# NoSuchThingAsRandom/EpidemicSimulator

Hardware: AMD Instinct MI355X
Metric: citizen-timesteps/sec (higher is better)
Workload: dtype u32 citizen word; u32 uniform vs ceil(q*2^32) (reference: f64 uniform; tolerance 2^-32 per draw); 1 GPU; uk64m: 64000000 citizens, 290000 Output Areas, 10 seeds, steps 1..667 of 5000, interventions on; seed=1592598545

## Files before the change

epidemicsimulator_amd/_lib.py:

```python
import ctypes as C
import os

_HERE = os.path.dirname(os.path.abspath(__file__))
LIB_PATH = os.environ.get("ESIM_LIB") or os.path.join(_HERE, "libesim.so")

OK = 0
ERRORS = {-1: "EINVAL", -2: "ENODEVICE", -3: "ENOMEM", -4: "ESTATE", -5: "ERANGE", -6: "ESIM", -7: "ETIMEDOUT"}

SUSCEPTIBLE, EXPOSED, INFECTED, RECOVERED, VACCINATED = range(5)
HOUSEHOLD, WORKPLACE, SCHOOL = range(3)
MASK_NONE, MASK_PUBLIC_TRANSPORT, MASK_EVERYWHERE = range(3)
NO_ROOM = 0xFFFFFFFF
FLAG_USES_PUBLIC_TRANSPORT = 1
FLAG_MASK_COMPLIANT = 2


class EsimError(RuntimeError):
    def __init__(self, code, text):
        super().__init__("libesim %s (%d): %s" % (ERRORS.get(code, "?"), code, text))
        self.code = code


class Params(C.Structure):
    _fields_ = [
# ... 8 lines not shown


_u32p, _u16p, _u8p, _i32p = (C.POINTER(C.c_uint32), C.POINTER(C.c_uint16),
                             C.POINTER(C.c_uint8), C.POINTER(C.c_int32))


class PopulationStruct(C.Structure):
    _fields_ = [
        ("n_citizens", C.c_uint32), ("n_buildings", C.c_uint32), ("n_areas", C.c_uint32),
        ("n_rooms", C.c_uint32), ("n_seeds", C.c_uint32),
        ("citizen_id_base", C.c_uint32), ("n_citizens_global", C.c_uint32),
        ("n_shared_buildings", C.c_uint32), ("n_shared_rooms", C.c_uint32),
        ("home_building", _u32p), ("work_building", _u32p), ("room", _u32p),
        ("flags", _u8p), ("age", _u16p), ("occupation", _u8p),
        ("building_area", _u32p), ("building_type", _u8p), ("room_building", _u32p),
        ("seeds", _u32p), ("shared_building_local", _i32p), ("shared_room_local", _i32p),
    ]


class StepResult(C.Structure):
    _fields_ = [(n, C.c_uint32) for n in (
        "time_step", "susceptible", "exposed", "infected", "recovered", "vaccinated",
        "exposures_building", "exposures_bus", "lockdown", "vaccination_active", "mask_status",
        "n_riders", "vaccinated_now", "eligible_count", "disease_exists", "reserved")]

    def as_dict(self):
        return {n: int(getattr(self, n)) for n, _ in self._fields_ if n != "reserved"}


RECORD_FIELDS = [n for n, _ in StepResult._fields_]


class SynthSpec(C.Structure):
    _fields_ = [
        ("n_citizens", C.c_uint32), ("n_areas", C.c_uint32), ("citizens_per_school", C.c_uint32),
        ("n_seeds", C.c_uint32), ("seed", C.c_uint64), ("area_jitter", C.c_double),
        ("p_public_transport", C.c_double), ("p_mask_compliant", C.c_double),
        ("p_work_from_home", C.c_double), ("p_teaching", C.c_double),
        ("household_buildings_median", C.c_double), ("household_buildings_sigma", C.c_double),
        ("p_area_without_households", C.c_double),
        ("workplace_buildings_median", C.c_double), ("workplace_buildings_sigma", C.c_double),
        ("p_area_without_workplaces", C.c_double),
        ("workplace_floor_median", C.c_double), ("workplace_floor_sigma", C.c_double),
        ("teacher_candidate_schools", C.c_uint32), ("reserved", C.c_uint32),
    ]


SYMBOLS = [
    "esim_default_params", "esim_create", "esim_upload_population", "esim_reset", "esim_restart", "esim_restart_seeded", "esim_get_seeds", "esim_step",
    "esim_run", "esim_set_pipeline", "esim_chunk_timing", "esim_enable_chunk_kernel_timing", "esim_chunk_kernel_timings", "esim_vax_chunk_stats", "esim_vax_repair_stats", "esim_pipeline_timing",
    "esim_comm_unique_id", "esim_comm_init_rccl", "esim_comm_init_callback", "esim_comm_set_timeout", "esim_debug_inject_error", "esim_comm_stats", "esim_run_sharded", "esim_shard_stats",
    "esim_read_records", "esim_synchronize",
    "esim_download_state", "esim_download_exposure_log", "esim_area_census", "esim_area_arrival", "esim_area_series", "esim_area_status_series", "esim_set_groups", "esim_group_census", "esim_group_series", "esim_ensemble_begin", "esim_ensemble_begin_arrival", "esim_ensemble_fold", "esim_ensemble_read", "esim_checkpoint_size", "esim_checkpoint_save", "esim_checkpoint_restore", "esim_enable_phase_timing", "esim_phase_timings",
    "esim_enable_kernel_timing", "esim_kernel_timings", "esim_set_small_step_limit", "esim_set_tiny_chunk_limit", "esim_small_kernel_timing", "esim_debug_counters",
    "esim_last_error", "esim_destroy",
    "esim_threshold_lut", "esim_synth_preset", "esim_synth_create", "esim_synth_create_shard", "esim_synth_free",
    "esim_shard_population", "esim_shard_cuts",
]

ALLREDUCE_FN = C.CFUNCTYPE(C.c_int, C.c_void_p, C.c_int, C.c_void_p, C.c_size_t)

_lib = None


def load():
    global _lib
    if _lib is not None:
        return _lib
    if not os.path.exists(LIB_PATH):
        raise ImportError(
            "libesim.so is not built (%s). Run `python -c 'import __graft_entry__ as g; g.build()'` "
            "or `make -C epidemicsimulator_amd/csrc`. There is no CPU fallback." % LIB_PATH)
    lib = C.CDLL(LIB_PATH)
    vp, pvp = C.c_void_p, C.POINTER(C.c_void_p)
    sig = {
        "esim_default_params": (None, [C.POINTER(Params)]),
        "esim_create": (C.c_int, [C.POINTER(Params), pvp]),
        "esim_upload_population": (C.c_int, [vp, C.POINTER(PopulationStruct)]),
        "esim_reset": (C.c_int, [vp]),
        "esim_restart": (C.c_int, [vp, C.POINTER(Params)]),
        "esim_restart_seeded": (C.c_int, [vp, C.POINTER(Params), _u32p, C.c_uint32]),
        "esim_get_seeds": (C.c_int, [vp, _u32p, C.c_uint32, _u32p]),
        "esim_step": (C.c_int, [vp, C.POINTER(StepResult)]),
        "esim_run": (C.c_int, [vp, C.c_uint32, C.c_int, C.POINTER(StepResult), C.POINTER(C.c_uint32)]),
        "esim_comm_unique_id": (C.c_int, [vp, C.c_size_t]),
        "esim_comm_init_rccl": (C.c_int, [vp, vp, C.c_size_t, C.c_int, C.c_int]),
        "esim_comm_init_callback": (C.c_int, [vp, ALLREDUCE_FN, vp, C.c_int, C.c_int]),
        "esim_comm_set_timeout": (C.c_int, [vp, C.c_double]),
        "esim_debug_inject_error": (C.c_int, [vp, C.c_int]),
        "esim_comm_stats": (C.c_int, [vp, C.POINTER(C.c_uint64)]),
        "esim_run_sharded": (C.c_int, [vp, C.c_uint32, C.POINTER(C.c_uint32)]),
        "esim_shard_stats": (C.c_int, [vp, C.POINTER(C.c_uint64), C.POINTER(C.c_uint64)]),
        "esim_set_pipeline": (C.c_int, [vp, C.c_int]),
        "esim_chunk_timing": (C.c_int, [vp, C.POINTER(C.c_double), C.POINTER(C.c_uint64), C.POINTER(C.c_uint64)]),
        "esim_enable_chunk_kernel_timing": (C.c_int, [vp, C.c_int]),
        "esim_chunk_kernel_timings": (C.c_int, [vp, C.POINTER(C.c_double), C.POINTER(C.c_uint64)]),
        "esim_vax_chunk_stats": (C.c_int, [vp, C.POINTER(C.c_uint64), C.POINTER(C.c_uint64)]),
        "esim_vax_repair_stats": (C.c_int, [vp, C.POINTER(C.c_uint64)]),
        "esim_pipeline_timing": (C.c_int, [vp, C.POINTER(C.c_double), C.POINTER(C.c_uint64), C.POINTER(C.c_uint64)]),
        "esim_read_records": (C.c_int, [vp, C.c_uint32, C.c_uint32, C.POINTER(StepResult)]),
        "esim_synchronize": (C.c_int, [vp]),
        "esim_download_state": (C.c_int, [vp, _u8p, _u16p, _u32p, _u8p, _u8p]),
        "esim_download_exposure_log": (C.c_int, [vp, _u32p, _u32p, _u8p, C.c_uint32, _u32p]),
        "esim_area_census": (C.c_int, [vp, C.c_int, _u32p]),
        "esim_area_arrival": (C.c_int, [vp, C.c_int, _u32p]),
        "esim_area_series": (C.c_int, [vp, C.c_int, C.c_uint32, C.c_uint32, C.c_uint32, _u32p]),
        "esim_area_status_series": (C.c_int, [vp, C.c_int, C.c_int, C.c_uint32, C.c_uint32, C.c_uint32, _u32p]),
        "esim_set_groups": (C.c_int, [vp, _u16p, C.c_uint32]),
        "esim_group_census": (C.c_int, [vp, _u32p]),
        "esim_group_series": (C.c_int, [vp, C.c_int, C.c_uint32, C.c_uint32, C.c_uint32, _u32p]),
        "esim_ensemble_begin": (C.c_int, [vp, C.c_int, C.c_uint32, C.c_uint32]),
        "esim_ensemble_begin_arrival": (C.c_int, [vp, C.c_int, C.c_uint32]),
        "esim_ensemble_fold": (C.c_int, [vp]),
        "esim_ensemble_read": (C.c_int, [vp, _u32p, _u32p, C.POINTER(C.c_uint64), C.POINTER(C.c_uint64)]),
        "esim_checkpoint_size": (C.c_int, [vp, C.POINTER(C.c_size_t)]),
        "esim_checkpoint_save": (C.c_int, [vp, vp, C.c_size_t]),
        "esim_checkpoint_restore": (C.c_int, [vp, vp, C.c_size_t]),
        "esim_enable_phase_timing": (C.c_int, [vp, C.c_int]),
        "esim_phase_timings": (C.c_int, [vp, C.POINTER(C.c_double)]),
        "esim_enable_kernel_timing": (C.c_int, [vp, C.c_int]),
        "esim_kernel_timings": (C.c_int, [vp, C.POINTER(C.c_double), C.POINTER(C.c_uint32)]),
        "esim_debug_counters": (C.c_int, [vp, C.POINTER(C.c_uint32)]),
        "esim_set_small_step_limit": (C.c_int, [vp, C.c_uint32]),
        "esim_set_tiny_chunk_limit": (C.c_int, [vp, C.c_uint32]),
        "esim_small_kernel_timing": (C.c_int, [vp, C.POINTER(C.c_double), C.POINTER(C.c_uint64)]),
        "esim_last_error": (C.c_char_p, [vp]),
        "esim_destroy": (None, [vp]),
        "esim_threshold_lut": (C.c_int, [C.POINTER(Params), C.POINTER(C.c_uint64)]),
        "esim_synth_preset": (C.c_int, [C.c_char_p, C.POINTER(SynthSpec)]),
        "esim_synth_create": (C.c_int, [C.POINTER(SynthSpec), C.POINTER(PopulationStruct)]),
        "esim_synth_create_shard": (C.c_int, [C.POINTER(SynthSpec), C.c_uint32, C.c_uint32, C.POINTER(PopulationStruct)]),
        "esim_shard_cuts": (C.c_int, [C.POINTER(PopulationStruct), C.c_uint32, C.c_int, C.POINTER(C.c_uint32)]),
        "esim_synth_free": (None, [C.POINTER(PopulationStruct)]),
        "esim_shard_population": (C.c_int, [C.POINTER(PopulationStruct), _u32p, C.c_uint32, C.c_uint32,
                                            C.POINTER(PopulationStruct)]),
    }
    for name, (res, args) in sig.items():
        fn = getattr(lib, name)
        fn.restype, fn.argtypes = res, args
    _lib = lib
    return lib


ESIM_OK, ESIM_ERANGE = 0, -5
AREA_CURRENT, AREA_HOME = 0, 1
SERIES_INFECTED, SERIES_EXPOSURES = 0, 1
BY_GROUP = 2
MAX_GROUPS = 1024
NEVER = 0xFFFFFFFF
GROUP_SERIES_EXPOSURES = 5
AREA_SERIES_INCIDENCE = 5
DEBUG_COUNTERS = ("t", "chunk_ok", "chunk_parallel", "chunk_pairs", "n_items", "items_per_wave", "n_units", "chunk_bus",
                  "n_route_pairs_big", "n_newexp", "log_len", "n_susceptible", "lockdown", "mask", "at_work", "bus_dir")
CHUNK_KERNELS = ("marks", "fold", "draw", "units", "count", "books", "scatter", "vax", "vax_adj", "vax_final", "decide", "future", "map_clear", "tiny", "vax_repair")
PHASE_OF_KERNEL = {"marks": "Generate Exposures", "fold": "Generate Exposures", "draw": "Apply Exposures", "units": "Apply Exposures"}
TINY_PHASE_SHARES = {"Generate Exposures": 0.10, "Apply Exposures": 0.40, "Apply Interventions": 0.50}


def check(code, ctx=None):
    if code != OK:
        text = load().esim_last_error(ctx)
        raise EsimError(code, text.decode() if text else "")


def default_params(**overrides):
    p = Params()
    load().esim_default_params(C.byref(p))
    for k, v in overrides.items():
        if not hasattr(p, k):
            raise AttributeError("esim_params has no field %r" % k)
        setattr(p, k, v)
    return p
```

epidemicsimulator_amd/csrc/esim_host_timing.h:

```cpp
extern "C" int esim_vax_chunk_stats(esim_ctx *ctx, uint64_t *steps, uint64_t *cuts)
{
    esim_ctx_impl *c = CTX(ctx); if (!c) return ESIM_EINVAL;
    if (steps) *steps = c->vax_chunk_steps;
    if (cuts) *cuts = c->vax_chunk_cuts;
    return ESIM_OK;
}

extern "C" int esim_vax_repair_stats(esim_ctx *ctx, uint64_t *repairs)
{
    esim_ctx_impl *c = CTX(ctx); if (!c) return ESIM_EINVAL;
    if (repairs) *repairs = c->vax_chunk_repairs;
    return ESIM_OK;
}

extern "C" int esim_chunk_timing(esim_ctx *ctx, double *total_ms, uint64_t *steps, uint64_t *chunks)
{
    esim_ctx_impl *c = CTX(ctx); if (!c) return ESIM_EINVAL;
    if (total_ms) *total_ms = c->tm.chunk_ms;
    if (steps) *steps = c->tm.chunk_steps;
    if (chunks) *chunks = c->tm.chunk_count;
    c->tm.chunk_ms = 0; c->tm.chunk_steps = 0; c->tm.chunk_count = 0;
    return ESIM_OK;
}

extern "C" int esim_enable_chunk_kernel_timing(esim_ctx *ctx, int enable)
{
    esim_ctx_impl *c = CTX(ctx); if (!c) return ESIM_EINVAL;
    if (int rc = drain(c)) return rc;
    c->tm.kdetail = enable != 0;
    c->tm.kd_used = 0;
    for (int i = 0; i < ESIM_CK_N; ++i) { c->tm.kd_ms[i] = 0; c->tm.kd_calls[i] = 0; }
    return ESIM_OK;
}

extern "C" int esim_chunk_kernel_timings(esim_ctx *ctx, double ms[ESIM_CK_N], uint64_t calls[ESIM_CK_N])
{
    esim_ctx_impl *c = CTX(ctx);
    if (!c || !ms || !calls) return ESIM_EINVAL;
    if (int rc = drain(c)) return rc;
    kd_resolve(c);
    for (int i = 0; i < ESIM_CK_N; ++i) { ms[i] = c->tm.kd_ms[i]; calls[i] = c->tm.kd_calls[i]; c->tm.kd_ms[i] = 0; c->tm.kd_calls[i] = 0; }
    return ESIM_OK;
}

extern "C" int esim_pipeline_timing(esim_ctx *ctx, double *mean_step_ms, uint64_t *steps_timed, uint64_t *steps_run)
{
    esim_ctx_impl *c = CTX(ctx); if (!c) return ESIM_EINVAL;
    if (int rc = drain(c)) return rc;
    double acc = 0;
    const size_t n = c->tm.pkev_used / 2;
    for (size_t i = 0; i < n; ++i) { float ms; HIP_TRY(c, hipEventElapsedTime(&ms, c->tm.pkev[2 * i], c->tm.pkev[2 * i + 1])); acc += ms; }
    if (mean_step_ms) *mean_step_ms = n ? acc / (double)n : 0.0;
    if (steps_timed) *steps_timed = n;
    if (steps_run) *steps_run = c->tm.pipe_steps;
    c->tm.pkev_used = 0; c->tm.pipe_steps = 0;
    return ESIM_OK;
}

extern "C" int esim_debug_counters(esim_ctx *ctx, uint32_t out[16])
{
    esim_ctx_impl *c = CTX(ctx);
    if (!c || !c->uploaded || !out) return ESIM_EINVAL;
    HIP_TRY(c, hipSetDevice(c->P.device));
    Ctrl h;
    const int rc = read_ctrl(c, &h);
    if (rc) return rc;
    const uint32_t v[16] = { h.t, h.chunk_ok, h.chunk_parallel, h.chunk_pairs, h.n_items, h.items_per_wave, h.n_units, h.chunk_bus,
                             h.n_route_pairs_big, h.n_newexp, h.log_len, h.n_susceptible, h.lockdown, h.mask, h.at_work, h.bus_dir };
    std::memcpy(out, v, sizeof v);
    return ESIM_OK;
}

#ifdef ESIM_COUNT_WORK
extern "C" int esim_work_counters(esim_ctx *ctx, unsigned long long *out, uint32_t n)
{
    esim_ctx_impl *c = CTX(ctx);
    if (!c || !c->uploaded || !out) return ESIM_EINVAL;
    if (int rc = drain(c)) return rc;
    unsigned long long h[WK_N];
    HIP_TRY(c, hipMemcpy(h, c->d.work_cnt, sizeof h, hipMemcpyDeviceToHost));
    HIP_TRY(c, hipMemset(c->d.work_cnt, 0, sizeof h));
    for (uint32_t i = 0; i < n; ++i) out[i] = i < WK_N ? h[i] : 0ull;
    return ESIM_OK;
}
#endif

#ifdef ESIM_WAVE_PROFILE
extern "C" int esim_prof_read(esim_ctx *ctx, uint32_t *out, uint32_t n_words, int *clock_khz)
{
    esim_ctx_impl *c = CTX(ctx);
    if (!c || !c->uploaded || !out) return ESIM_EINVAL;
    if (int rc = drain(c)) return rc;
    HIP_TRY(c, hipMemcpy(out, c->d.prof_buf, sizeof(uint32_t) * std::min<uint32_t>(n_words, 16384u * 16u), hipMemcpyDeviceToHost));
    if (clock_khz) HIP_TRY(c, hipDeviceGetAttribute(clock_khz, hipDeviceAttributeWallClockRate, c->P.device));
    return ESIM_OK;
}
#endif

extern "C" int esim_enable_phase_timing(esim_ctx *ctx, int enable)
{
    esim_ctx_impl *c = CTX(ctx); if (!c) return ESIM_EINVAL;
    c->tm.phase = enable != 0;
    return ESIM_OK;
}

extern "C" int esim_phase_timings(esim_ctx *ctx, double out[4])
{
    esim_ctx_impl *c = CTX(ctx);
    if (!c || !out) return ESIM_EINVAL;
    out[0] = c->tm.phase_s[0]; out[1] = c->tm.phase_s[1]; out[2] = c->tm.phase_s[2];
    out[3] = out[0] + out[1] + out[2];
    return ESIM_OK;
}

extern "C" int esim_enable_kernel_timing(esim_ctx *ctx, int enable)
{
    esim_ctx_impl *c = CTX(ctx); if (!c) return ESIM_EINVAL;
    c->tm.kernel = enable > 0;
    if (enable > 0) c->tm.stride = (uint32_t)enable;
    c->tm.kev_used = 0;
    if (enable > 0) {
        HIP_TRY(c, hipSetDevice(c->P.device));
// ... 28 lines not shown
```

epidemicsimulator_amd/csrc/esim_kernels_chunk.h:

```cpp
#pragma once
#define BF_WIN 1024
__device__ __forceinline__ void block_scan_1024(uint32_t *v, uint32_t *wtmp)
{
    const uint32_t tid = threadIdx.x, lane = tid & 63u, wv = tid >> 6;
    uint32_t x = v[tid];
#pragma unroll
    for (int o = 1; o < 64; o <<= 1) { const uint32_t y = __shfl_up(x, o, 64); if (lane >= (uint32_t)o) x += y; }
    if (lane == 63u) wtmp[wv] = x;
    __syncthreads();
    if (tid == 0) { uint32_t a = 0; for (uint32_t w = 0; w < FIN_TPB / 64; ++w) { const uint32_t y = wtmp[w]; wtmp[w] = a; a += y; } }
    __syncthreads();
    v[tid] = x + wtmp[wv];
    __syncthreads();
}

__device__ __forceinline__ void future_body(const Dev &d, uint32_t max_ahead, uint32_t limit_t, uint32_t *win, uint32_t *wtmp)
{
    Ctrl *ctrl = d.ctrl;
    const uint32_t t0 = ld(&ctrl->t), tid = threadIdx.x;
    const uint32_t n_ahead = t0 > limit_t ? 0u : (limit_t - t0 + 1u < max_ahead ? limit_t - t0 + 1u : max_ahead);
    const int et = (int)d.exposed_time, it = (int)d.infected_time;
    const int base_idx = (int)(t0 + TE_BIAS) - et - 1 - it;
    { const int k = base_idx + (int)tid; win[tid] = (k >= 0 && k < (int)TE_SLOTS) ? ld(&d.hist[k]) : 0u; }
    __syncthreads();
// ... 1136 lines not shown
{
    ItemFetch f;
    f.slot = FX(x, LANE_HSLOT); f.id = FX(x, 0); f.a_lo = FX(x, 1); f.a_hi = FX(x, 2); f.b_lo = FX(x, 3); f.b_hi = FX(x, 4); f.aux = FX(x, 5); f.link = FX(x, 6);
    f.c0 = 0u; f.c1 = 0u;
    if (f.slot < d.hcap) {
        item_counts(d, x, f.slot, lane, n, AW, BUS, f.c0, f.c1);
        iv_count(FX(x, 7), lane, AW, BUS, f.c0, f.c1);
    }
    return f;
}

__device__ __forceinline__ bool item_ok(const Dev &d, const ItemFetch &it)
{
    if (it.slot >= d.hcap) return false;
    if (it.id < d.n_bld) return it.a_lo <= it.a_hi && it.a_hi <= d.n && it.b_lo <= it.b_hi && it.b_hi <= d.n_wrk_idx;
    if (it.id < d.n_bld + d.n_room) return it.a_lo <= it.a_hi && it.a_hi <= d.n_room_idx && (it.link == 0xFFFFFFFFu || it.link < d.hcap);
    return true;
}
#define PAIR_SPREAD 1237u
__device__ __forceinline__ void route_pair_small(const Dev &d, Ctrl *ctrl, const ChunkShared &sm, uint32_t off, uint32_t sz, uint32_t j, uint32_t t0, uint32_t lane WORK_ARG)
{
    const uint64_t seed = ((uint64_t)d.seed_hi << 32) | d.seed_lo;
    const uint32_t s = t0 + j, mask = sm.dec[j].mask;
    uint32_t c = 0, w = 0, key = 0;
    bool inf = false;
    WORK_ADD(WK_ROUTE_PAIRS, lane == 0 ? 1 : 0); WORK_ADD(WK_RIDERS, lane < sz ? 1 : 0);
    bool can = false;
    if (lane < sz) {
        c = d.route_riders[off + lane];
        w = d.cit[c];
        inf = status_in_chunk(d, w, t0, j) == ESIM_INFECTED;
        const uint32_t te = CW_TE(w);
        can = !(w <= CW_MAKE(s + TE_BIAS, CW_BUS_EXPOSED | (w & CW_KEEP)) || (te >= TE_RECOVERED && te != TE_SUSCEPTIBLE) || j > CW_VAX_REL(w));
    }
    if (!__any(inf) || !__any(can)) return;
    uint32_t rank = 0;
    if (sz > d.bus_capacity) {
        if (lane < sz) key = philox4x32_10(d.id_base + c, s, ESIM_SLOT_BUS_ORDER, 0u, d.seed_lo, d.seed_hi).w0;
        for (uint32_t i = 0; i < sz; ++i) {
            const uint32_t ki = (uint32_t)__builtin_amdgcn_readlane((int)key, (int)i);
            rank += ki < key || (ki == key && i < lane);
        }
    }
    const uint32_t bus = rank / d.bus_capacity;
    const unsigned long long inf_m = __ballot(inf);
    uint32_t k = 0;
    const uint32_t n_bus = (sz + d.bus_capacity - 1u) / d.bus_capacity;
    for (uint32_t b = 0; b < n_bus; ++b) {
        const unsigned long long on_b = __ballot(lane < sz && bus == b);
        if (bus == b) k = (uint32_t)__popcll(on_b & inf_m);
    }
    if (lane < sz && k && can) {
        const uint32_t row = (!(w & FL_MASK_COMPLIANT) && mask == ESIM_MASK_EVERYWHERE) ? 1u : 0u;
        WORK_ADD(WK_BUS_DRAWS, 1);
        if (esim_u32(seed, d.id_base + c, s, ESIM_SLOT_BUS) < sm.thr[row * 256u + (k & 255u)]) { WORK_ADD(WK_HITS, 1); expose_min(d, ctrl, c, w, s, CW_BUS_EXPOSED); }
    }
}

template <uint32_t NT>
__device__ __forceinline__ void route_pair_big(const Dev &d, Ctrl *ctrl, const ChunkShared &sm, RouteShared &rs, uint32_t code, uint32_t t0, uint32_t n WORK_ARG)
{
    const uint64_t seed = ((uint64_t)d.seed_hi << 32) | d.seed_lo;
    const uint32_t r = code >> 7, j = code & 127u;
    if (r >= d.n_routes || j >= n) { if (threadIdx.x == 0) ctrl->error = (uint32_t)(-ESIM_ERANGE); return; }
    const uint32_t off = d.route_off[r], sz = d.route_off[r + 1] - off;
    if (sz > CHUNK_ROUTE_MAX) { if (threadIdx.x == 0) ctrl->error = (uint32_t)(-ESIM_ERANGE); return; }
    const uint32_t s = t0 + j, mask = sm.dec[j].mask;
    WORK_ADD(WK_ROUTE_PAIRS, threadIdx.x == 0 ? 1 : 0);
    int loc_inf = 0, loc_can = 0;
    for (uint32_t i = threadIdx.x; i < sz; i += NT) {
        const uint32_t c = d.route_riders[off + i];
        WORK_ADD(WK_RIDERS, 1);
        const uint32_t w = d.cit[c], te = CW_TE(w);
        rs.s_inf[i] = status_in_chunk(d, w, t0, j) == ESIM_INFECTED ? 1 : 0;
        loc_inf |= rs.s_inf[i];
        loc_can |= !(w <= CW_MAKE(s + TE_BIAS, CW_BUS_EXPOSED | (w & CW_KEEP)) || (te >= TE_RECOVERED && te != TE_SUSCEPTIBLE) || j > CW_VAX_REL(w)) ? 1 : 0;
    }
    const int any_inf = __syncthreads_or(loc_inf), any_can = __syncthreads_or(loc_can);
    if (!any_inf || !any_can) return;
    for (uint32_t i = threadIdx.x; i < sz; i += NT)
        rs.s_key[i] = philox4x32_10(d.id_base + d.route_riders[off + i], s, ESIM_SLOT_BUS_ORDER, 0u, d.seed_lo, d.seed_hi).w0;
    for (uint32_t i = threadIdx.x; i < sz / d.bus_capacity + 1u; i += NT) rs.s_cnt[i] = 0u;
    __syncthreads();
    for (uint32_t i = threadIdx.x; i < sz; i += NT) {
        const uint32_t ki = rs.s_key[i];
        uint32_t rank = 0;
        for (uint32_t qq = 0; qq < sz; ++qq) { const uint32_t kq = rs.s_key[qq]; rank += kq < ki || (kq == ki && qq < i); }
        const uint32_t bus = rank / d.bus_capacity;
        rs.s_bus[i] = (uint16_t)bus;
        if (rs.s_inf[i]) atomicAdd(&rs.s_cnt[bus], 1u);
    }
    __syncthreads();
    for (uint32_t i = threadIdx.x; i < sz; i += NT) {
        const uint32_t k = rs.s_cnt[rs.s_bus[i]];
        if (!k) continue;
        const uint32_t c = d.route_riders[off + i];
        const uint32_t w = d.cit[c], te = CW_TE(w);
        if (w <= CW_MAKE(s + TE_BIAS, CW_BUS_EXPOSED | (w & CW_KEEP)) || (te >= TE_RECOVERED && te != TE_SUSCEPTIBLE) || j > CW_VAX_REL(w)) continue;
        const uint32_t row = (!(w & FL_MASK_COMPLIANT) && mask == ESIM_MASK_EVERYWHERE) ? 1u : 0u;
        WORK_ADD(WK_BUS_DRAWS, 1);
        if (esim_u32(seed, d.id_base + c, s, ESIM_SLOT_BUS) < sm.thr[row * 256u + (k & 255u)]) { WORK_ADD(WK_HITS, 1); expose_min(d, ctrl, c, w, s, CW_BUS_EXPOSED); }
    }
    __syncthreads();
}

__global__ __launch_bounds__(TPB) void k_chunk_draw(Dev d, uint32_t n_mw)
// ... 69 lines not shown
        if (v + 1u < d_hi) sl_cur = fetch_slot(d, FX(id_cur, LANE_HSLOT), lane);
        const uint32_t pq0 = PROF_NOW();
        const ItemFetch it = decode_item(d, x, lane, n, AW, BUS);
        if (it.slot == ITEM_UNUSED) continue;
        if (!item_ok(d, it)) { if (lane == 0) RAISE(ctrl, ESIM_ERANGE, ERR_AT_ITEM_CHECK); continue; }
        if (it.id >= route_base) continue;
        const uint32_t pi0 = PROF_NOW();
        pst[0] += pi0 - pq0;
        (void)pi0; ++p_items; WORK_ADD(WK_ITEMS, lane == 0 ? 1 : 0);
        if (it.id < d.n_bld) {
            if (it.aux == ESIM_SCHOOL) continue;
            const uint32_t n_res = it.a_hi - it.a_lo, n_wrk = it.b_hi - it.b_lo;
            uint32_t rm = 0u, wm = 0u, rw = 0u, ww = 0u;
            if (lane < n_res) rm = d.res_idx ? d.res_idx[it.a_lo + lane] : it.a_lo + lane;
            if (lane < n_wrk) wm = d.wrk_idx[it.b_lo + lane];
            if (lane < n_res) rw = d.cit[rm];
            if (lane < n_wrk) ww = d.cit[wm];
            const uint32_t pq1 = PROF_NOW();
            const uint32_t S = item_steps_regs(it.c0, it.c1, lane, ws, t0, AW, EV);
            __builtin_amdgcn_wave_barrier();
            const uint32_t pq2 = PROF_NOW();
            const UnitSrc src = { it.slot, it.link, FX(x, 7) };
            list_or_units(d, ctrl, sm, ws, d.res_idx, it.a_lo, it.a_hi, src, lane, 0u, S, t0 WORK_PASS, true, rm, rw);
            const uint32_t pq3 = PROF_NOW();
            list_or_units(d, ctrl, sm, ws, d.wrk_idx, it.b_lo, it.b_hi, src, lane, 1u, S, t0 WORK_PASS, true, wm, ww);
            const uint32_t pq4 = PROF_NOW();
            pst[1] += pq1 - pi0; pst[2] += pq2 - pq1; pst[3] += pq3 - pq2; pst[4] += pq4 - pq3;
        } else {
            const uint32_t n_mem = it.a_hi - it.a_lo;
            uint32_t mm = 0u, mw = 0u;
            if (lane < n_mem) mm = d.room_idx[it.a_lo + lane];
            school_counts(d, it.link, lane, n, q0, q1, ws);
            if (lane < n_mem) mw = d.cit[mm];
            const uint32_t S = item_steps_regs(it.c0, it.c1, lane, ws, t0, AW, EV);
            __builtin_amdgcn_wave_barrier();
            const UnitSrc src = { it.slot, it.link, FX(x, 7) };
            list_or_units(d, ctrl, sm, ws, d.room_idx, it.a_lo, it.a_hi, src, lane, 2u, S, t0 WORK_PASS, true, mm, mw);
        }
        __builtin_amdgcn_wave_barrier();
        { const uint32_t dt = PROF_NOW() - pi0; p_item_max = dt > p_item_max ? dt : p_item_max; }
    }
    const uint32_t pt2 = PROF_NOW();
    for (uint32_t k0 = 0; k0 * G < K; k0 += 64u) {
        if (k0) {
            const uint32_t kk = (k0 + lane) * G + w_rep;
            have = false;
            if (kk < K) {
                const uint32_t src = (w_base + n_mw - (uint32_t)(((unsigned long long)kk * PAIR_SPREAD) % n_mw)) % n_mw;
                code_l = d.route_pairs[(size_t)src * K + kk];
                have = kk < d.pair_cnt[src] && (code_l >> 7) < d.n_routes && (code_l & 127u) < n;
            }
            if (have) { const uint32_t r = code_l >> 7; off_l = d.route_off[r]; sz_l = d.route_off[r + 1] - off_l; }
        }
        unsigned long long todo = __ballot(have);
        while (todo) {
            const int src_lane = __ffsll((long long)todo) - 1;
            todo &= todo - 1ull;
            const uint32_t code = __shfl(code_l, src_lane, 64), off = __shfl(off_l, src_lane, 64), sz = __shfl(sz_l, src_lane, 64);
            route_pair_small(d, ctrl, sm, off, sz, code & 127u, t0, lane WORK_PASS);
        }
    }
    WORK_FLUSH(d);
    const uint32_t pt3 = PROF_NOW();
#ifndef ESIM_PROFILE_UNITS
    PROF_PUT(d, 0, pt0); PROF_PUT(d, 1, pt1); PROF_PUT(d, 2, pt2); PROF_PUT(d, 3, pt3);
    PROF_PUT(d, 4, p_items); PROF_PUT(d, 5, p_item_max); PROF_PUT(d, 6, wsc[threadIdx.x >> 6].rounds);
    PROF_PUT(d, 11, pst[0]); PROF_PUT(d, 12, pst[1]); PROF_PUT(d, 13, pst[2]); PROF_PUT(d, 14, pst[3]); PROF_PUT(d, 15, pst[4]);
#endif
    (void)pst;
    (void)pt0; (void)pt1; (void)pt2; (void)pt3; (void)p_items; (void)p_item_max;
}

__global__ __launch_bounds__(TPB) void k_chunk_units(Dev d)
{
    __shared__ ChunkShared sm;
    __shared__ WaveScratch wsc[TPB / 64];
    __shared__ RouteShared rs;
    Ctrl *ctrl = d.ctrl;
    const uint32_t t0 = ctrl->chunk_t0, n = ctrl->chunk_ok;
    if (!ctrl->chunk_parallel || n == 0u) return;
    const uint32_t lane = threadIdx.x & 63u;
    const uint32_t wave = (blockIdx.x * TPB + threadIdx.x) >> 6, n_waves = (gridDim.x * TPB) >> 6;
    const uint32_t pu0 = PROF_NOW();
    WORK_TALLY;
    uint32_t pu_n = 0u, pu_max = 0u, pu_it = 0u;
    const uint32_t qr = wave & (SUBQ - 1u), first = wave / SUBQ, step = n_waves / SUBQ;
    const uint32_t n_units = step ? min(ld(&d.hot[(HOT_UNITS + qr) * HOT_STRIDE]), d.unit_qcap) : 0u;
    const uint32_t n_pairs = min(ld(&d.hot[HOT_BIGPAIRS * HOT_STRIDE]), d.big_pairs_cap);
    if (__syncthreads_or(first < n_units) == 0 && n_pairs == 0u) return;
    for (uint32_t i = threadIdx.x; i < n; i += TPB) sm.dec[i] = d.dec[i];
    for (uint32_t i = threadIdx.x; i < 512u; i += TPB) sm.thr[i] = d.thr[i];
    __syncthreads();
    WaveScratch &ws = wsc[threadIdx.x >> 6];
    const uint32_t *q_words = reinterpret_cast<const uint32_t *>(d.units + (size_t)qr * d.unit_qcap);
    const Decision q0 = lane < n ? sm.dec[lane] : Decision{ 0u, 0u, 0u, 0u };
    const Decision q1 = 64u + lane < n ? sm.dec[64u + lane] : Decision{ 0u, 0u, 0u, 0u };
    M96 AW, BUS;
    schedule_masks(lane, n, q0, q1, AW, BUS);
    const M96 EV = { __ballot(lane < n && q0.mask == ESIM_MASK_EVERYWHERE), (uint32_t)__ballot(64u + lane < n && q1.mask == ESIM_MASK_EVERYWHERE) };
    auto unit_words = [&](uint32_t q) -> uint32_t { return lane < 8u ? q_words[(size_t)q * 8u + lane] : 0u; };
    auto member_id = [&](uint32_t u) -> uint32_t {
        const uint32_t code = FX(u, 4), kind = code >> 30, lo = FX(u, 2), n_mem = FX(u, 3), mf = FX(u, 6);
        if (code == UNIT_NOOP || mf + lane >= n_mem) return 0u;
        const uint32_t *idx = kind == 2u ? d.room_idx : kind == 1u ? d.wrk_idx : d.res_idx;
        return idx ? idx[lo + mf + lane] : lo + mf + lane;
    };
    const uint32_t pu1 = PROF_NOW();
    uint32_t u_0 = 0xFFFFFFFFu, u_1 = 0xFFFFFFFFu;
    uint32_t xs_0 = 0u, ys_0 = 0u, mid_0 = 0u;
    if (first < n_units) u_0 = unit_words(first);
    if (first + step < n_units) u_1 = unit_words(first + step);
    if (first < n_units && FX(u_0, 4) != UNIT_NOOP) { xs_0 = fetch_slot(d, FX(u_0, 0), lane); ys_0 = fetch_slot(d, FX(u_0, 1), lane); mid_0 = member_id(u_0); }
    for (uint32_t q = first; q < n_units; q += step) {
        const uint32_t u = u_0, xs = xs_0, ys = ys_0, mid = mid_0;
        u_0 = u_1;
        u_1 = 0xFFFFFFFFu;
        if (q + 2u * step < n_units) u_1 = unit_words(q + 2u * step);
        if (q + step < n_units && FX(u_0, 4) != UNIT_NOOP) { xs_0 = fetch_slot(d, FX(u_0, 0), lane); ys_0 = fetch_slot(d, FX(u_0, 1), lane); mid_0 = member_id(u_0); }
        const uint32_t code = FX(u, 4);
        if (code == UNIT_NOOP) continue;
        const uint32_t pui = PROF_NOW();
        ++pu_n;
        const uint32_t kind = code >> 30, p_lo = code & 0x3FFFFFFFu, slot = FX(u, 0), link = FX(u, 1), lo = FX(u, 2), n_mem = FX(u, 3), own = FX(u, 5), mf = FX(u, 6);
// ... 367 lines not shown
```

epidemicsimulator_amd/csrc/esim_kernels_common.h:

```cpp
#pragma once
#include <hip/hip_runtime.h>
#include "../../include/esim.h"
#include "esim_device.h"
#include "philox.h"

#define TPB 256
#define FIN_TPB 1024

__device__ __forceinline__ uint32_t status_of(uint32_t te, uint32_t t, uint32_t et, uint32_t it)
{
    if (te == TE_SUSCEPTIBLE) return ESIM_SUSCEPTIBLE;
    if (te == TE_VACCINATED) return ESIM_VACCINATED;
    if (te == TE_RECOVERED) return ESIM_RECOVERED;
    uint32_t d = t + TE_BIAS - te;
    if (d <= et) return ESIM_EXPOSED;
    if (d <= et + 1u + it) return ESIM_INFECTED;
    return ESIM_RECOVERED;
}

__device__ __forceinline__ uint32_t ld(const uint32_t *p)
{
    return __hip_atomic_load(p, __ATOMIC_RELAXED, __HIP_MEMORY_SCOPE_AGENT);
}

// ... 39 lines not shown
    for (int k = lo_i + (int)threadIdx.x; k <= hi_e; k += (int)blockDim.x) {
        if (k < 0) continue;
        const uint32_t v = ld(&d.hist[k]);
        if (k >= lo_e) e += v; else i += v;
    }
    if (e) atomicAdd(&out[1], e);
    if (i) atomicAdd(&out[2], i);
    __syncthreads();
    if (threadIdx.x == 0) {
        out[0] = ld(&ctrl->n_susceptible); out[4] = ld(&ctrl->n_vaccinated);
        out[3] = d.n - out[0] - out[4] - out[1] - out[2];
    }
    __syncthreads();
}

__device__ __forceinline__ void append(uint32_t *list, uint32_t *len, uint32_t v)
{
    list[atomicAdd(len, 1u)] = v;
}

#ifdef ESIM_WAVE_PROFILE
#define PROF_ROW 16u
#define PROF_NOW() ((uint32_t)wall_clock64())
#define PROF_PUT(d, i, v) do { if ((threadIdx.x & 63u) == 0) (d).prof_buf[(size_t)(((blockIdx.x * TPB + threadIdx.x) >> 6)) * PROF_ROW + (i)] = (uint32_t)(v); } while (0)
#define BOOKS_PROF(d, i, v) do { if (threadIdx.x == 0) (d).prof_buf[(size_t)16383 * PROF_ROW + (i)] = (uint32_t)(v); } while (0)
#define TINY_PROF(d, i) do { if (threadIdx.x == 0) (d).prof_buf[(size_t)16382 * PROF_ROW + (i)] = (uint32_t)wall_clock64(); } while (0)
#else
#define BOOKS_PROF(d, i, v) do { (void)sizeof(v); } while (0)
#define TINY_PROF(d, i) do { } while (0)
#define PROF_NOW() 0u
#define PROF_PUT(d, i, v) do { (void)sizeof(v); } while (0)
#endif


#ifdef ESIM_COUNT_WORK
enum { WK_ENTRIES = 0,
       WK_KEYS,
       WK_CLAIMS,
       WK_RECORDS,
       WK_DIRECT,
       WK_FOLDED,
       WK_ITEMS,
       WK_MEMBERS,
       WK_MEMBERS_IDX,
       WK_PAIRS,
       WK_PAIRS_ACTIVE,
       WK_BLOCKS,
       WK_DRAWS,
       WK_UNITS,
       WK_ROUTE_PAIRS,
       WK_RIDERS,
       WK_BUS_DRAWS,
       WK_HITS,
       WK_N };
#define WORK_TALLY uint32_t wk_[WK_N]; for (int wk_i = 0; wk_i < WK_N; ++wk_i) wk_[wk_i] = 0u
#define WORK_ADD(i, x) (wk_[i] += (uint32_t)(x))
#define WORK_FLUSH(d) do { for (int wk_i = 0; wk_i < WK_N; ++wk_i) { uint32_t x_ = wk_[wk_i]; for (int o_ = 32; o_ > 0; o_ >>= 1) x_ += __shfl_xor(x_, o_, 64); \
        if ((threadIdx.x & 63u) == 0 && x_) atomicAdd(&(d).work_cnt[wk_i], (unsigned long long)x_); wk_[wk_i] = 0u; } } while (0)
#define WORK_ARG , uint32_t *wk_
#define WORK_PASS , wk_
#else
#define WORK_TALLY do { } while (0)
#define WORK_ADD(i, x) do { } while (0)
#define WORK_FLUSH(d) do { } while (0)
#define WORK_ARG
#define WORK_PASS
#endif
```

include/esim.h:

```cpp
#ifndef ESIM_H
#define ESIM_H
#include <stddef.h>
#include <stdint.h>

#ifdef __cplusplus
extern "C" {
#endif

#define ESIM_OK          0
#define ESIM_EINVAL     -1
#define ESIM_ENODEVICE  -2
#define ESIM_ENOMEM     -3
#define ESIM_ESTATE     -4
#define ESIM_ERANGE     -5
#define ESIM_ESIM       -6
#define ESIM_ETIMEDOUT  -7

enum { ESIM_SUSCEPTIBLE = 0, ESIM_EXPOSED = 1, ESIM_INFECTED = 2, ESIM_RECOVERED = 3, ESIM_VACCINATED = 4 };
enum { ESIM_HOUSEHOLD = 0, ESIM_WORKPLACE = 1, ESIM_SCHOOL = 2 };
enum { ESIM_MASK_NONE = 0, ESIM_MASK_PUBLIC_TRANSPORT = 1, ESIM_MASK_EVERYWHERE = 2 };

#define ESIM_NO_ROOM 0xFFFFFFFFu
#define ESIM_FLAG_USES_PUBLIC_TRANSPORT 1u
#define ESIM_FLAG_MASK_COMPLIANT        2u
// ... 77 lines not shown
int  esim_set_pipeline(esim_ctx *ctx, int level);
int  esim_chunk_timing(esim_ctx *ctx, double *total_ms, uint64_t *steps, uint64_t *chunks);
enum { ESIM_CK_MARKS = 0, ESIM_CK_FOLD, ESIM_CK_DRAW, ESIM_CK_UNITS, ESIM_CK_COUNT, ESIM_CK_BOOKS, ESIM_CK_SCATTER, ESIM_CK_VAX, ESIM_CK_VAX_ADJ,
       ESIM_CK_VAX_FINAL, ESIM_CK_DECIDE, ESIM_CK_FUTURE, ESIM_CK_MAP_CLEAR, ESIM_CK_TINY, ESIM_CK_VAX_REPAIR, ESIM_CK_N };
int  esim_enable_chunk_kernel_timing(esim_ctx *ctx, int enable);
int  esim_chunk_kernel_timings(esim_ctx *ctx, double ms[ESIM_CK_N], uint64_t calls[ESIM_CK_N]);
int  esim_vax_chunk_stats(esim_ctx *ctx, uint64_t *steps, uint64_t *cuts);
int  esim_vax_repair_stats(esim_ctx *ctx, uint64_t *repairs);
int  esim_read_records(esim_ctx *ctx, uint32_t first_step, uint32_t n, esim_step_result *out);
int  esim_synchronize(esim_ctx *ctx);

int  esim_download_state(esim_ctx *ctx, uint8_t *status, uint16_t *timer,
                         uint32_t *current_building, uint8_t *on_bus, uint8_t *eligible);
int  esim_download_exposure_log(esim_ctx *ctx, uint32_t *citizen, uint32_t *step, uint8_t *on_bus, uint32_t cap, uint32_t *n_out);
enum { ESIM_AREA_CURRENT = 0, ESIM_AREA_HOME = 1 };
int  esim_area_census(esim_ctx *ctx, int where, uint32_t *counts );
#define ESIM_NEVER 0xFFFFFFFFu
int  esim_area_arrival(esim_ctx *ctx, int where, uint32_t *step_out );
int  esim_ensemble_begin(esim_ctx *ctx, int where, uint32_t status_mask, uint32_t min_cases);
int  esim_ensemble_begin_arrival(esim_ctx *ctx, int where, uint32_t horizon);
int  esim_ensemble_fold(esim_ctx *ctx);
int  esim_ensemble_read(esim_ctx *ctx, uint32_t *members, uint32_t *hit ,
                        uint64_t *sum , uint64_t *sumsq );
enum { ESIM_SERIES_INFECTED = 0, ESIM_SERIES_EXPOSURES = 1 };
int  esim_area_series(esim_ctx *ctx, int what, uint32_t first_step, uint32_t n_rows, uint32_t stride,
                      uint32_t *out );
enum { ESIM_AREA_SERIES_INCIDENCE = 5 };
int  esim_area_status_series(esim_ctx *ctx, int where, int what, uint32_t first_step, uint32_t n_rows, uint32_t stride,
                             uint32_t *out );
#define ESIM_MAX_GROUPS 1024
enum { ESIM_BY_GROUP = 2 };
enum { ESIM_GROUP_SERIES_EXPOSURES = 5 };
int  esim_set_groups(esim_ctx *ctx, const uint16_t *group , uint32_t n_groups);
int  esim_group_census(esim_ctx *ctx, uint32_t *counts );
int  esim_group_series(esim_ctx *ctx, int what, uint32_t first_step, uint32_t n_rows, uint32_t stride,
                       uint32_t *out );
int  esim_checkpoint_size(esim_ctx *ctx, size_t *bytes);
int  esim_checkpoint_save(esim_ctx *ctx, void *buf, size_t cap);
int  esim_checkpoint_restore(esim_ctx *ctx, const void *buf, size_t bytes);

int  esim_enable_phase_timing(esim_ctx *ctx, int enable);
int  esim_phase_timings(esim_ctx *ctx, double out[4]);

int  esim_enable_kernel_timing(esim_ctx *ctx, int enable);
int  esim_kernel_timings(esim_ctx *ctx, double *step_ms, uint32_t *out_n);

int  esim_set_small_step_limit(esim_ctx *ctx, uint32_t max_infected);
int  esim_small_kernel_timing(esim_ctx *ctx, double *total_ms, uint64_t *steps);
int  esim_set_tiny_chunk_limit(esim_ctx *ctx, uint32_t max_pairs);
int  esim_pipeline_timing(esim_ctx *ctx, double *mean_step_ms, uint64_t *steps_timed, uint64_t *steps_run);

int  esim_debug_counters(esim_ctx *ctx, uint32_t out[16]);

const char *esim_last_error(const esim_ctx *ctx);
void esim_destroy(esim_ctx *ctx);

int  esim_threshold_lut(const esim_params *p, uint64_t out[512]);

typedef struct esim_synth_spec {
    uint32_t n_citizens, n_areas, citizens_per_school, n_seeds;
    uint64_t seed;
    double   area_jitter;
    double   p_public_transport, p_mask_compliant;
    double   p_work_from_home;
    double   p_teaching;
    double   household_buildings_median, household_buildings_sigma;
    double   p_area_without_households;
    double   workplace_buildings_median, workplace_buildings_sigma;
    double   p_area_without_workplaces;
    double   workplace_floor_median, workplace_floor_sigma;
    uint32_t teacher_candidate_schools;
    uint32_t reserved;
} esim_synth_spec;
int  esim_synth_preset(const char *name, esim_synth_spec *out);
int  esim_synth_create(const esim_synth_spec *spec, esim_population *out);
int  esim_synth_create_shard(const esim_synth_spec *spec, uint32_t shard, uint32_t n_shards, esim_population *out);
void esim_synth_free(esim_population *pop);
int  esim_shard_population(const esim_population *whole, const uint32_t *cuts, uint32_t n_shards,
                           uint32_t shard, esim_population *out);
int  esim_shard_cuts(const esim_population *whole, uint32_t n_shards, int by_work, uint32_t *cuts_out);

#ifdef __cplusplus
}
#endif
#endif
```

Baseline: 52810 billion citizen-timesteps/s.

## Pack multiple small bus route pairs into one wavefront pass

Replaces the per-route serial loop, where the whole wave processed one rider group at a time, with a packed scheme. A prefix sum lays several route segments (each at most 64 riders) across the 64 lanes, and each segment is handled by its own lanes. Ranking for over-capacity buses uses segmented bpermute comparisons, with a fallback to an exact tie-break when keys collide. A debug entry point and extra work counters are added to test the segmented ranking. This adds complexity and cross-lane shuffles, and uses a new check for whether a segment is live.

```diff
diff --git a/epidemicsimulator_amd/_lib.py b/epidemicsimulator_amd/_lib.py
--- a/epidemicsimulator_amd/_lib.py
+++ b/epidemicsimulator_amd/_lib.py
@@ -84,7 +84,7 @@
     "esim_comm_unique_id", "esim_comm_init_rccl", "esim_comm_init_callback", "esim_comm_set_timeout", "esim_debug_inject_error", "esim_comm_stats", "esim_run_sharded", "esim_shard_stats",
     "esim_read_records", "esim_synchronize",
     "esim_download_state", "esim_download_exposure_log", "esim_area_census", "esim_area_arrival", "esim_area_series", "esim_area_status_series", "esim_set_groups", "esim_group_census", "esim_group_series", "esim_ensemble_begin", "esim_ensemble_begin_arrival", "esim_ensemble_fold", "esim_ensemble_read", "esim_checkpoint_size", "esim_checkpoint_save", "esim_checkpoint_restore", "esim_enable_phase_timing", "esim_phase_timings",
-    "esim_enable_kernel_timing", "esim_kernel_timings", "esim_set_small_step_limit", "esim_set_tiny_chunk_limit", "esim_small_kernel_timing", "esim_debug_counters",
+    "esim_enable_kernel_timing", "esim_kernel_timings", "esim_set_small_step_limit", "esim_set_tiny_chunk_limit", "esim_small_kernel_timing", "esim_debug_counters", "esim_debug_seg_ranks",
     "esim_last_error", "esim_destroy",
     "esim_threshold_lut", "esim_synth_preset", "esim_synth_create", "esim_synth_create_shard", "esim_synth_free",
     "esim_shard_population", "esim_shard_cuts",
@@ -153,6 +153,7 @@
         "esim_enable_kernel_timing": (C.c_int, [vp, C.c_int]),
         "esim_kernel_timings": (C.c_int, [vp, C.POINTER(C.c_double), C.POINTER(C.c_uint32)]),
         "esim_debug_counters": (C.c_int, [vp, C.POINTER(C.c_uint32)]),
+        "esim_debug_seg_ranks": (C.c_int, [vp, _u32p, _u32p, C.c_uint32, _u32p, _u32p]),
         "esim_set_small_step_limit": (C.c_int, [vp, C.c_uint32]),
         "esim_set_tiny_chunk_limit": (C.c_int, [vp, C.c_uint32]),
         "esim_small_kernel_timing": (C.c_int, [vp, C.POINTER(C.c_double), C.POINTER(C.c_uint64)]),
diff --git a/epidemicsimulator_amd/csrc/esim_host_timing.h b/epidemicsimulator_amd/csrc/esim_host_timing.h
--- a/epidemicsimulator_amd/csrc/esim_host_timing.h
+++ b/epidemicsimulator_amd/csrc/esim_host_timing.h
@@ -68,6 +68,29 @@
     const uint32_t v[16] = { h.t, h.chunk_ok, h.chunk_parallel, h.chunk_pairs, h.n_items, h.items_per_wave, h.n_units, h.chunk_bus,
                              h.n_route_pairs_big, h.n_newexp, h.log_len, h.n_susceptible, h.lockdown, h.mask, h.at_work, h.bus_dir };
     std::memcpy(out, v, sizeof v);
+    return ESIM_OK;
+}
+
+extern "C" int esim_debug_seg_ranks(esim_ctx *ctx, const uint32_t *keys, const uint32_t *seg_sizes, uint32_t n_seg, uint32_t *ranks, uint32_t *tied)
+{
+    esim_ctx_impl *c = CTX(ctx);
+    if (!c || !keys || !seg_sizes || !ranks || !tied || n_seg == 0 || n_seg > 64) return ESIM_EINVAL;
+    uint32_t h[193] = { 0 }, lanes = 0;
+    for (uint32_t q = 0; q < n_seg; ++q) {
+        if (seg_sizes[q] == 0 || seg_sizes[q] > 64u - lanes) return fail(c, ESIM_EINVAL, "esim_debug_seg_ranks: segments of 1 .. 64 lanes, 64 in all at most");
+        h[64 + q] = seg_sizes[q]; lanes += seg_sizes[q];
+    }
+    std::memcpy(h, keys, sizeof(uint32_t) * lanes);
+    if (int rc = drain(c)) return rc;
+    DevTmp<uint32_t> buf;
+    HIP_TRY(c, buf.alloc(193));
+    HIP_TRY(c, hipMemcpy(buf.p, h, sizeof h, hipMemcpyHostToDevice));
+    hipLaunchKernelGGL(k_debug_seg_ranks, dim3(1), dim3(64), 0, c->stream, buf.p, n_seg);
+    HIP_TRY(c, hipGetLastError());
+    HIP_TRY(c, hipStreamSynchronize(c->stream));
+    HIP_TRY(c, hipMemcpy(h, buf.p, sizeof h, hipMemcpyDeviceToHost));
+    std::memcpy(ranks, h + 128, sizeof(uint32_t) * lanes);
+    *tied = h[192];
     return ESIM_OK;
 }
 
diff --git a/epidemicsimulator_amd/csrc/esim_kernels_chunk.h b/epidemicsimulator_amd/csrc/esim_kernels_chunk.h
--- a/epidemicsimulator_amd/csrc/esim_kernels_chunk.h
+++ b/epidemicsimulator_amd/csrc/esim_kernels_chunk.h
@@ -1212,6 +1212,97 @@
     }
     if (lane < sz && k && can) {
         const uint32_t row = (!(w & FL_MASK_COMPLIANT) && mask == ESIM_MASK_EVERYWHERE) ? 1u : 0u;
+        WORK_ADD(WK_BUS_DRAWS, 1);
+        if (esim_u32(seed, d.id_base + c, s, ESIM_SLOT_BUS) < sm.thr[row * 256u + (k & 255u)]) { WORK_ADD(WK_HITS, 1); expose_min(d, ctrl, c, w, s, CW_BUS_EXPOSED); }
+    }
+}
+
+template <bool EXACT>
+__device__ __forceinline__ uint32_t seg_count_less(uint32_t key, uint32_t lane, uint32_t base, uint32_t sz, uint32_t n_iter)
+{
+    uint32_t rank = 0;
+    if (EXACT) {
+        for (uint32_t i = 0; i < n_iter; ++i) {
+            const uint32_t ki = (uint32_t)__builtin_amdgcn_ds_bpermute((int)((base + i) << 2), (int)key);
+            rank += i < sz && (ki < key || (ki == key && base + i < lane)) ? 1u : 0u;
+        }
+        return rank;
+    }
+    for (uint32_t i = 0; i < n_iter; i += 4u) {
+        uint32_t ki[4];
+#pragma unroll
+        for (uint32_t u = 0; u < 4u; ++u) ki[u] = (uint32_t)__builtin_amdgcn_ds_bpermute((int)((base + i + u) << 2), (int)key);
+#pragma unroll
+        for (uint32_t u = 0; u < 4u; ++u) rank += i + u < sz && ki[u] < key ? 1u : 0u;
+    }
+    return rank;
+}
+
+__device__ __forceinline__ uint32_t seg_ranks(uint32_t key, uint32_t lane, uint32_t base, uint32_t sz, uint32_t n_iter, bool &tied)
+{
+    uint32_t rank = seg_count_less<false>(key, lane, base, sz, n_iter);
+    const uint32_t got = (uint32_t)__builtin_amdgcn_ds_permute((int)((sz ? base + rank : lane) << 2), 1);
+    tied = __any(sz && !got);
+    if (tied) rank = seg_count_less<true>(key, lane, base, sz, n_iter);
+    return rank;
+}
+
+__device__ __forceinline__ void route_pairs_packed(const Dev &d, Ctrl *ctrl, const ChunkShared &sm, unsigned long long batch, uint32_t code_l, uint32_t off_l,
+                                                   uint32_t sz_l, uint32_t start_l, uint32_t t0, uint32_t lane WORK_ARG)
+{
+    const uint64_t seed = ((uint64_t)d.seed_hi << 32) | d.seed_lo;
+    const uint32_t cap = d.bus_capacity;
+    uint32_t src = 0u;
+    for (unsigned long long m = batch; m; m &= m - 1ull) {
+        const int p = __builtin_ctzll(m);
+        if (lane >= (uint32_t)__builtin_amdgcn_readlane((int)start_l, p)) src = (uint32_t)p;
+    }
+    const int last = 63 - __builtin_clzll(batch);
+    const uint32_t total = (uint32_t)__builtin_amdgcn_readlane((int)start_l, last) + (uint32_t)__builtin_amdgcn_readlane((int)sz_l, last);
+    const bool valid = lane < total;
+    const uint32_t base = __shfl(start_l, (int)src, 64), code = __shfl(code_l, (int)src, 64), off = __shfl(off_l, (int)src, 64);
+    const uint32_t sz = valid ? __shfl(sz_l, (int)src, 64) : 0u;
+    const unsigned long long seg = (sz >= 64u ? ~0ull : (1ull << sz) - 1ull) << (base & 63u);
+    const uint32_t j = code & 127u, s = t0 + j;
+    uint32_t c = 0, w = 0;
+    bool inf = false, can = false;
+    WORK_ADD(WK_ROUTE_BATCHES, lane == 0 ? 1 : 0); WORK_ADD(WK_ROUTE_PAIRS, valid && lane == base ? 1 : 0); WORK_ADD(WK_RIDERS, valid ? 1 : 0);
+    if (valid) {
+        c = d.route_riders[off + (lane - base)];
+        w = d.cit[c];
+        inf = status_in_chunk(d, w, t0, j) == ESIM_INFECTED;
+        const uint32_t te = CW_TE(w);
+        can = !(w <= CW_MAKE(s + TE_BIAS, CW_BUS_EXPOSED | (w & CW_KEEP)) || (te >= TE_RECOVERED && te != TE_SUSCEPTIBLE) || j > CW_VAX_REL(w));
+    }
+    const unsigned long long inf_m = __ballot(inf), can_m = __ballot(can);
+    const bool live = (inf_m & seg) != 0ull && (can_m & seg) != 0ull;
+    WORK_ADD(WK_ROUTE_PAIRS_LIVE, live && lane == base ? 1 : 0);
+    if (!__any(live)) return;
+    const uint32_t sz_r = live && sz > cap ? sz : 0u;
+    uint32_t rank = 0u, n_iter = 0u;
+    for (unsigned long long m = __ballot(sz_r && lane == base); m; m &= m - 1ull) {
+        const uint32_t z = (uint32_t)__builtin_amdgcn_readlane((int)sz_r, __builtin_ctzll(m));
+        n_iter = z > n_iter ? z : n_iter;
+    }
+    if (n_iter) {
+        uint32_t key = 0u;
+        bool tied;
+        WORK_ADD(WK_ROUTE_PAIRS_RANKED, sz_r && lane == base ? 1 : 0); WORK_ADD(WK_ROUTE_KEY_ISSUES, lane == 0 ? 1 : 0);
+        if (sz_r) key = philox4x32_10(d.id_base + c, s, ESIM_SLOT_BUS_ORDER, 0u, d.seed_lo, d.seed_hi).w0;
+        rank = seg_ranks(key, lane, base, sz_r, n_iter, tied);
+    }
+    uint32_t k = 0u;
+    for (uint32_t lo = 0u; lo < (n_iter ? n_iter : 1u); lo += cap) {
+        const bool on = live && rank - lo < cap;
+        const unsigned long long on_b = __ballot(on);
+        if (on) k = (uint32_t)__popcll(on_b & inf_m & seg);
+    }
+    const bool draw = live && k && can;
+#ifdef ESIM_COUNT_WORK
+    { const unsigned long long dm = __ballot(draw); WORK_ADD(WK_ROUTE_PAIRS_DRAWING, valid && lane == base && (dm & seg) ? 1 : 0); WORK_ADD(WK_ROUTE_DRAW_ISSUES, lane == 0 && dm ? 1 : 0); }
+#endif
+    if (draw) {
+        const uint32_t row = (!(w & FL_MASK_COMPLIANT) && sm.dec[j].mask == ESIM_MASK_EVERYWHERE) ? 1u : 0u;
         WORK_ADD(WK_BUS_DRAWS, 1);
         if (esim_u32(seed, d.id_base + c, s, ESIM_SLOT_BUS) < sm.thr[row * 256u + (k & 255u)]) { WORK_ADD(WK_HITS, 1); expose_min(d, ctrl, c, w, s, CW_BUS_EXPOSED); }
     }
@@ -1387,12 +1478,17 @@
             }
             if (have) { const uint32_t r = code_l >> 7; off_l = d.route_off[r]; sz_l = d.route_off[r + 1] - off_l; }
         }
+        have = have && sz_l <= 64u;
+        const uint32_t n_l = have ? sz_l : 0u;
+        uint32_t incl = n_l;
+        for (uint32_t o = 1u; o < 64u; o <<= 1) { const uint32_t up = __shfl_up(incl, o, 64); if (lane >= o) incl += up; }
         unsigned long long todo = __ballot(have);
+        uint32_t taken = 0u;
         while (todo) {
-            const int src_lane = __ffsll((long long)todo) - 1;
-            todo &= todo - 1ull;
-            const uint32_t code = __shfl(code_l, src_lane, 64), off = __shfl(off_l, src_lane, 64), sz = __shfl(sz_l, src_lane, 64);
-            route_pair_small(d, ctrl, sm, off, sz, code & 127u, t0, lane WORK_PASS);
+            const unsigned long long batch = __ballot(have && incl - taken <= 64u) & todo;
+            route_pairs_packed(d, ctrl, sm, batch, code_l, off_l, sz_l, incl - n_l - taken, t0, lane WORK_PASS);
+            todo &= ~batch;
+            taken = (uint32_t)__builtin_amdgcn_readlane((int)incl, 63 - __builtin_clzll(batch));
         }
     }
     WORK_FLUSH(d);
@@ -1404,6 +1500,22 @@
 #endif
     (void)pst;
     (void)pt0; (void)pt1; (void)pt2; (void)pt3; (void)p_items; (void)p_item_max;
+}
+
+__global__ __launch_bounds__(64) void k_debug_seg_ranks(uint32_t *buf, uint32_t n_seg)
+{
+    const uint32_t lane = threadIdx.x & 63u;
+    uint32_t base = 0u, sz = 0u, n_iter = 0u, at = 0u;
+    for (uint32_t q = 0; q < n_seg && q < 64u; ++q) {
+        const uint32_t z = buf[64u + q];
+        if (lane >= at && lane - at < z) { base = at; sz = z; }
+        at += z;
+        n_iter = z > n_iter ? z : n_iter;
+    }
+    bool tied;
+    const uint32_t rank = seg_ranks(buf[lane], lane, base, sz, n_iter, tied);
+    buf[128u + lane] = rank;
+    if (lane == 0) buf[192u] = tied ? 1u : 0u;
 }
 
 __global__ __launch_bounds__(TPB) void k_chunk_units(Dev d)
diff --git a/epidemicsimulator_amd/csrc/esim_kernels_common.h b/epidemicsimulator_amd/csrc/esim_kernels_common.h
--- a/epidemicsimulator_amd/csrc/esim_kernels_common.h
+++ b/epidemicsimulator_amd/csrc/esim_kernels_common.h
@@ -115,6 +115,12 @@
        WK_RIDERS,
        WK_BUS_DRAWS,
        WK_HITS,
+       WK_ROUTE_BATCHES,
+       WK_ROUTE_PAIRS_LIVE,
+       WK_ROUTE_PAIRS_RANKED,
+       WK_ROUTE_PAIRS_DRAWING,
+       WK_ROUTE_KEY_ISSUES,
+       WK_ROUTE_DRAW_ISSUES,
        WK_N };
 #define WORK_TALLY uint32_t wk_[WK_N]; for (int wk_i = 0; wk_i < WK_N; ++wk_i) wk_[wk_i] = 0u
 #define WORK_ADD(i, x) (wk_[i] += (uint32_t)(x))
diff --git a/include/esim.h b/include/esim.h
--- a/include/esim.h
+++ b/include/esim.h
@@ -153,6 +153,8 @@
 
 int  esim_debug_counters(esim_ctx *ctx, uint32_t out[16]);
 
+int  esim_debug_seg_ranks(esim_ctx *ctx, const uint32_t *keys, const uint32_t *seg_sizes, uint32_t n_seg, uint32_t *ranks, uint32_t *tied);
+
 const char *esim_last_error(const esim_ctx *ctx);
 void esim_destroy(esim_ctx *ctx);
 
```

Result: no change. 52610 billion citizen-timesteps/s (-0.4%).
